# myscience/open-genie

Measured on NVIDIA H100. Metric: videotokenizer_train_step_frames_per_sec, higher is better.
Workload: dtype bf16

## Files before the change

open_genie_b200/csrc/conv3d_wgrad.cu:

```cuda
#include "og_host.cuh"
#include "og_ptx.cuh"

namespace og {
extern std::atomic<uint64_t> g_launches;

static constexpr int kWThreads = 384;
static constexpr int kVox = 64;
static constexpr int kPanelBytes = kVox * 128;
static constexpr int kTileM = 128;
static constexpr int kTileN = 256;
static constexpr int kWABytes = 2 * kPanelBytes;
static constexpr int kWBBytes = 4 * kPanelBytes;
static constexpr int kWStages = 4;
static constexpr int kSlotFloats = kTileM * kTileN;

struct WgradParams {
  int kt, kh, kw, pt, ph, pw;
  int sx_t, sx_h, sx_w;
  int bw_log2, bh_log2, bt_log2, bn_log2;
  int tiles_w, tiles_h, tiles_t;
  int num_ksteps;
  int cin, cout;
  int ncols;
  int col_tiles;
  long long units;
  int ctas;
  int granule;
  int period;
  float* dw;
  long long ld_dw;
  int vec_ok;
  float* dbias;
  int n_bias;
  float* ws;
};

__host__ __device__ __forceinline__ long long share_begin(const WgradParams& p, int b) {
  return (long long)b * (p.units / p.granule) / p.ctas * p.granule;
}

template <bool kOnes>
__device__ __forceinline__ void wgrad_mma_steps(float (&acc)[128], float (&accb)[8], int nsteps, const uint8_t* smem_a,
                                                const uint8_t* smem_b, uint32_t ones_addr, uint64_t* full,
                                                uint64_t* empty, int& s, uint32_t& ph, int lane) {
  int prev = -1;
  for (int i = 0; i < nsteps; ++i) {
    mbar_wait(&full[s], ph);
    const uint32_t a_addr = smem_u32(smem_a + s * kWABytes);
    const uint32_t b_addr = smem_u32(smem_b + s * kWBBytes);
    wgmma_fence();
#pragma unroll
    for (int k = 0; k < kVox / 16; ++k)
      wgmma_ss<256, 1, 1>(acc, gmma_desc_sw128(a_addr + k * 2048, kPanelBytes, 1024),
                          gmma_desc_sw128(b_addr + k * 2048, kPanelBytes, 1024), (i | k) != 0);
    if constexpr (kOnes) {
#pragma unroll
      for (int k = 0; k < kVox / 16; ++k)
        wgmma_ss<16, 1, 1>(accb, gmma_desc_sw128(a_addr + k * 2048, kPanelBytes, 1024),
                           gmma_desc_sw128(ones_addr, kPanelBytes, 1024), (i | k) != 0);
    }
    wgmma_commit();
    wgmma_wait<1>();
    if (prev >= 0 && lane == 0) mbar_arrive(&empty[prev]);
    prev = s;
    if (++s == kWStages) {
      s = 0;
      ph ^= 1;
    }
  }
  wgmma_wait<0>();
  if (lane == 0) mbar_arrive(&empty[prev]);
}

template <bool kBias>
__global__ void __launch_bounds__(kWThreads, 1)
    og_conv_wgrad_kernel(const __grid_constant__ CUtensorMap mapDY, const __grid_constant__ CUtensorMap mapX,
                         const WgradParams p) {
  extern __shared__ uint8_t smem_raw[];
  uint8_t* smem = reinterpret_cast<uint8_t*>((reinterpret_cast<uintptr_t>(smem_raw) + 1023) & ~uintptr_t(1023));
  uint8_t* smem_a = smem;
  uint8_t* smem_b = smem + kWStages * kWABytes;
  uint8_t* smem_ones = smem_b + kWStages * kWBBytes;
  uint64_t* full = reinterpret_cast<uint64_t*>(smem_ones + 2048);
  uint64_t* empty = full + kWStages;

  const int warp = warp_idx_uniform();
  const int lane = threadIdx.x & 31;
  const long long u_begin = share_begin(p, blockIdx.x), u_end = share_begin(p, blockIdx.x + 1);

  if (warp == 0 && lane == 0) {
    tma_prefetch_desc(&mapDY);
    tma_prefetch_desc(&mapX);
    for (int s = 0; s < kWStages; ++s) {
      mbar_init(&full[s], 1);
      mbar_init(&empty[s], 8);
    }
    fence_mbar_init();
  }
  if (kBias) {
    for (int i = threadIdx.x; i < 2048 / 4; i += kWThreads) reinterpret_cast<uint32_t*>(smem_ones)[i] = 0x3F803F80u;
    fence_proxy_async_smem();
  }
  __syncthreads();

  if (warp == 0) {
    int s = 0;
    uint32_t ph = 0;
    const int per_sample = p.tiles_w * p.tiles_h * p.tiles_t;
    long long clock = 0;
    for (long long u = u_begin; u < u_end;) {
      const int tile = (int)(u / p.num_ksteps);
      const int k0 = (int)(u - (long long)tile * p.num_ksteps);
      const int k1 = (int)min((long long)p.num_ksteps, u_end - (long long)tile * p.num_ksteps);
      u += k1 - k0;
      const int co0 = (tile / p.col_tiles) * kTileM;
      const int c0 = (tile % p.col_tiles) * kTileN;
      const int npan = min(4, (p.ncols - c0) / 64);
      int pci[4], off_w[4], off_h[4], off_t[4];
#pragma unroll
      for (int j = 0; j < 4; ++j) {
        const int c = c0 + 64 * (j < npan ? j : 0);
        const int tap = c / p.cin;
        pci[j] = c - tap * p.cin;
        off_t[j] = tap / (p.kh * p.kw) - p.pt;
        off_h[j] = (tap / p.kw) % p.kh - p.ph;
        off_w[j] = tap % p.kw - p.pw;
      }
      const uint32_t tx_bytes = (uint32_t)(kWABytes + npan * kPanelBytes);
      int ks = k0 + (int)((clock - k0 % p.period + p.period) % p.period);
      if (ks >= k1) ks = k0;
      clock += k1 - k0;
      int tn, tw, th, tt;
      auto decode = [&](int k) {
        tn = k / per_sample;
        int r = k - tn * per_sample;
        tw = r % p.tiles_w;
        r /= p.tiles_w;
        th = r % p.tiles_h;
        tt = r / p.tiles_h;
      };
      decode(ks);
      for (int i = k0; i < k1; ++i) {
        const int n = tn << p.bn_log2, w0 = tw << p.bw_log2, h0 = th << p.bh_log2, t0 = tt << p.bt_log2;
        mbar_wait(&empty[s], ph ^ 1);
        if (elect_one()) {
          mbar_expect_tx(&full[s], tx_bytes);
          uint8_t* a = smem_a + s * kWABytes;
          tma_load_5d(a, &mapDY, &full[s], co0, w0, h0, t0, n);
          tma_load_5d(a + kPanelBytes, &mapDY, &full[s], co0 + 64, w0, h0, t0, n);
          uint8_t* b = smem_b + s * kWBBytes;
          for (int j = 0; j < npan; ++j)
            tma_load_5d(b + j * kPanelBytes, &mapX, &full[s], pci[j], w0 * p.sx_w + off_w[j], h0 * p.sx_h + off_h[j],
                        t0 * p.sx_t + off_t[j], n);
        }
        __syncwarp();
        if (++s == kWStages) {
          s = 0;
          ph ^= 1;
        }
        if (++ks == k1) {
          ks = k0;
          decode(ks);
        } else if (++tw == p.tiles_w) {
          tw = 0;
          if (++th == p.tiles_h) {
            th = 0;
            if (++tt == p.tiles_t) {
              tt = 0;
              ++tn;
            }
          }
        }
      }
    }
    __syncwarp();
  } else if (warp >= 4) {
    const int wg = (warp >> 2) - 1;
    const int q = warp & 3;
    const uint32_t ones_addr = smem_u32(smem_ones);
    const uint8_t* a_wg = smem_a + wg * kPanelBytes;
    float acc[128], accb[8];
    int s = 0;
    uint32_t ph = 0;
    for (long long u = u_begin; u < u_end;) {
      const bool first = u == u_begin;
      const int tile = (int)(u / p.num_ksteps);
      const int k0 = (int)(u - (long long)tile * p.num_ksteps);
      const int k1 = (int)min((long long)p.num_ksteps, u_end - (long long)tile * p.num_ksteps);
      u += k1 - k0;
      const int co0 = (tile / p.col_tiles) * kTileM;
      const int c0 = (tile % p.col_tiles) * kTileN;
      const bool bias_tile = kBias && c0 == 0;
      if (bias_tile)
        wgrad_mma_steps<true>(acc, accb, k1 - k0, a_wg, smem_b, ones_addr, full, empty, s, ph, lane);
      else
        wgrad_mma_steps<false>(acc, accb, k1 - k0, a_wg, smem_b, ones_addr, full, empty, s, ph, lane);
      reg_fence(acc);
      reg_fence(accb);
      const bool whole = k0 == 0 && k1 == p.num_ksteps;
      const int slot = 2 * blockIdx.x + (first ? 0 : 1);
      const int c_lane = 2 * (lane & 3);
#pragma unroll
      for (int rr = 0; rr < 2; ++rr) {
        const int r = wg * 64 + q * 16 + (lane >> 2) + rr * 8;
        const int co = co0 + r;
        if (whole) {
          if (co >= p.cout) continue;
          float* row = p.dw + (long long)co * p.ld_dw + c0 + c_lane;
#pragma unroll
          for (int j = 0; j < 32; ++j) {
            if (c0 + 8 * j + c_lane >= p.ncols) continue;
            const float v0 = acc[4 * j + 2 * rr], v1 = acc[4 * j + 2 * rr + 1];
            if (p.vec_ok) {
              float2* d = reinterpret_cast<float2*>(row + 8 * j);
              const float2 o = *d;
              *d = make_float2(o.x + v0, o.y + v1);
            } else {
              row[8 * j] += v0;
              row[8 * j + 1] += v1;
            }
          }
          if (bias_tile && (lane & 3) == 0 && co < p.n_bias) p.dbias[co] += accb[2 * rr];
        } else {
          float* sl = p.ws + ((long long)slot * kTileM + r) * kTileN + c_lane;
#pragma unroll
          for (int j = 0; j < 32; ++j)
            *reinterpret_cast<float2*>(sl + 8 * j) = make_float2(acc[4 * j + 2 * rr], acc[4 * j + 2 * rr + 1]);
          if (bias_tile && (lane & 3) == 0)
            p.ws[(long long)2 * p.ctas * kSlotFloats + (long long)slot * kTileM + r] = accb[2 * rr];
        }
      }
    }
  }
}

__global__ void __launch_bounds__(256) og_wgrad_fixup_kernel(const WgradParams p) {
  const int b = blockIdx.y;
  const long long ub = share_begin(p, b + 1);
  const int tile = (int)(ub / p.num_ksteps);
  const long long t0 = (long long)tile * p.num_ksteps, t1 = t0 + p.num_ksteps;
  if (ub == t0 || share_begin(p, b) > t0) return;
  const int co0 = (tile / p.col_tiles) * kTileM, c0 = (tile % p.col_tiles) * kTileN;
  const int e = (blockIdx.x * 256 + threadIdx.x) * 4;
  const int r = e / kTileN, c = e % kTileN;
  float4 sum = make_float4(0.f, 0.f, 0.f, 0.f);
  float sumb = 0.f;
  const bool bias = p.dbias && c0 == 0 && blockIdx.x == 0 && threadIdx.x < kTileM;
  for (int sh = b; sh < p.ctas; ++sh) {
    const long long sb = share_begin(p, sh);
    if (sb >= t1) break;
    const int slot = 2 * sh + (sb >= t0 ? 0 : 1);
    const float4 v = __ldcg(reinterpret_cast<const float4*>(p.ws + (long long)slot * kSlotFloats + e));
    sum.x += v.x;
    sum.y += v.y;
    sum.z += v.z;
    sum.w += v.w;
    if (bias) sumb += __ldcg(p.ws + (long long)2 * p.ctas * kSlotFloats + (long long)slot * kTileM + threadIdx.x);
  }
  if (co0 + r < p.cout && c0 + c < p.ncols) {
    float* d = p.dw + (long long)(co0 + r) * p.ld_dw + c0 + c;
    d[0] += sum.x;
    d[1] += sum.y;
    d[2] += sum.z;
    d[3] += sum.w;
  }
  if (bias && co0 + (int)threadIdx.x < p.n_bias) p.dbias[co0 + threadIdx.x] += sumb;
}

}

static int launch_wgrad(const void* dy, int cout, const void* x, int cin, float* dw, int64_t ld_dw, int kt, int kh, int kw,
                        int pt, int ph, int pw, int N, int T, int H, int W, int Ti, int Hi, int Wi, int st, int sh, int sw,
                        void* workspace, size_t workspace_bytes, og_stream_t stream, float* dbias = nullptr,
                        int n_bias = 0) {
  using namespace og;
  OG_REQUIRE(dy && x && dw, "conv3d_wgrad: null pointer");
  OG_REQUIRE(!dbias || (n_bias > 0 && n_bias <= cout), "conv3d_wgrad: n_bias=%d must be in 1..cout", n_bias);
  OG_REQUIRE(cin > 0 && cin % 64 == 0, "conv3d_wgrad: cin=%d must be a multiple of 64", cin);
  OG_REQUIRE(cout > 0 && cout % 8 == 0, "conv3d_wgrad: cout=%d must be a multiple of 8 (TMA row stride)", cout);
  OG_REQUIRE(kt >= 1 && kh >= 1 && kw >= 1 && pt >= 0 && ph >= 0 && pw >= 0 && pt < kt && ph < kh && pw < kw,
             "conv3d_wgrad: bad kernel/padding");
  OG_REQUIRE(st >= 1 && sh >= 1 && sw >= 1 && st <= 8 && sh <= 8 && sw <= 8, "conv3d_wgrad: bad stride");
  OG_REQUIRE(N > 0 && T > 0 && H > 0 && W > 0 && Ti > 0 && Hi > 0 && Wi > 0,
             "conv3d_wgrad: extents must be positive (N=%d T=%d H=%d W=%d)", N, T, H, W);
  OG_REQUIRE(ld_dw >= (int64_t)kt * kh * kw * cin, "conv3d_wgrad: ld_dw=%lld must be >= kt*kh*kw*cin = %d",
             (long long)ld_dw, kt * kh * kw * cin);
  int bw, bh, bt, bn;
  choose_voxel_box(kVox, N, T, H, W, &bw, &bh, &bt, &bn);
  OG_REQUIRE(bw * sw <= 256 && bh * sh <= 256 && bt * st <= 256, "conv3d_wgrad: strided box exceeds the TMA limit");
  WgradParams p;
  memset(&p, 0, sizeof(p));
  p.kt = kt; p.kh = kh; p.kw = kw; p.pt = pt; p.ph = ph; p.pw = pw;
  p.sx_t = st; p.sx_h = sh; p.sx_w = sw;
  p.bw_log2 = ilog2(bw); p.bh_log2 = ilog2(bh); p.bt_log2 = ilog2(bt); p.bn_log2 = ilog2(bn);
  p.tiles_w = (W + bw - 1) / bw; p.tiles_h = (H + bh - 1) / bh; p.tiles_t = (T + bt - 1) / bt;
  p.num_ksteps = ((N + bn - 1) / bn) * p.tiles_w * p.tiles_h * p.tiles_t;
  p.cin = cin; p.cout = cout; p.dw = dw; p.ld_dw = ld_dw;
  p.ncols = kt * kh * kw * cin;
  p.col_tiles = (p.ncols + kTileN - 1) / kTileN;
  const long long tiles = (long long)((cout + kTileM - 1) / kTileM) * p.col_tiles;
  p.units = tiles * p.num_ksteps;
  const int sms = num_sms();
  p.ctas = (int)std::min<long long>(sms, std::max<long long>(1, p.units / 4));
  p.granule = 1;
  const size_t slot_bytes = (size_t)(kSlotFloats + (dbias ? kTileM : 0)) * sizeof(float);
  const long long fit = workspace ? (long long)(workspace_bytes / (2 * slot_bytes)) : 0;
  if (fit < p.ctas) {
    if (fit > tiles) {
      p.ctas = (int)fit;
    } else {
      p.granule = p.num_ksteps;
      p.ctas = (int)std::min<long long>(sms, tiles);
    }
  }
  p.period = (int)std::min<long long>(p.num_ksteps, (p.units + p.ctas - 1) / p.ctas);
  p.ws = reinterpret_cast<float*>(workspace);
  p.vec_ok = (ld_dw % 2 == 0) && ((reinterpret_cast<uintptr_t>(dw) & 7) == 0);
  p.dbias = dbias;
  p.n_bias = n_bias;
  const size_t smem_bytes = (size_t)kWStages * (kWABytes + kWBBytes) + 2048  + 1024 + 512;

  CUtensorMap mapDY, mapX;
  {
    uint64_t dims[5] = {(uint64_t)cout, (uint64_t)W, (uint64_t)H, (uint64_t)T, (uint64_t)N};
    uint64_t str[4] = {(uint64_t)cout * 2, (uint64_t)W * cout * 2, (uint64_t)H * W * cout * 2,
                       (uint64_t)T * H * W * cout * 2};
    uint32_t box[5] = {64, (uint32_t)bw, (uint32_t)bh, (uint32_t)bt, (uint32_t)bn};
    int r = make_tmap_bf16(&mapDY, dy, 5, dims, str, box);
    if (r != OG_OK) return r;
  }
  {
    uint64_t dims[5] = {(uint64_t)cin, (uint64_t)Wi, (uint64_t)Hi, (uint64_t)Ti, (uint64_t)N};
    uint64_t str[4] = {(uint64_t)cin * 2, (uint64_t)Wi * cin * 2, (uint64_t)Hi * Wi * cin * 2,
                       (uint64_t)Ti * Hi * Wi * cin * 2};
    uint32_t box[5] = {64, (uint32_t)(bw * sw), (uint32_t)(bh * sh), (uint32_t)(bt * st), (uint32_t)bn};
    uint32_t es[5] = {1, (uint32_t)sw, (uint32_t)sh, (uint32_t)st, 1};
    int r = make_tmap_bf16(&mapX, x, 5, dims, str, box, es);
    if (r != OG_OK) return r;
  }
  static bool attr_set = false;
  if (!attr_set) {
    OG_CHECK_CUDA(cudaFuncSetAttribute(og_conv_wgrad_kernel<false>, cudaFuncAttributeMaxDynamicSharedMemorySize,
                                       (int)smem_bytes));
    OG_CHECK_CUDA(cudaFuncSetAttribute(og_conv_wgrad_kernel<true>, cudaFuncAttributeMaxDynamicSharedMemorySize,
                                       (int)smem_bytes));
    attr_set = true;
  }
  if (dbias)
    og_conv_wgrad_kernel<true><<<p.ctas, kWThreads, smem_bytes, (cudaStream_t)stream>>>(mapDY, mapX, p);
  else
    og_conv_wgrad_kernel<false><<<p.ctas, kWThreads, smem_bytes, (cudaStream_t)stream>>>(mapDY, mapX, p);
  OG_CHECK_CUDA(cudaGetLastError());
  g_launches.fetch_add(1);
  if (p.granule == 1 && p.ctas > 1) {
    og_wgrad_fixup_kernel<<<dim3(kSlotFloats / 1024, p.ctas - 1), 256, 0, (cudaStream_t)stream>>>(p);
    OG_CHECK_CUDA(cudaGetLastError());
    g_launches.fetch_add(1);
  }
  return OG_OK;
}

extern "C" int og_conv3d_wgrad(const void* dy, int cout, const void* x, int cin, float* dw, int64_t ld_dw, int kt,
                               int kh, int kw, int pt, int ph, int pw, int N, int T, int H, int W, void* workspace,
                               size_t workspace_bytes, og_stream_t stream) {
  return launch_wgrad(dy, cout, x, cin, dw, ld_dw, kt, kh, kw, pt, ph, pw, N, T, H, W, T, H, W, 1, 1, 1, workspace,
                      workspace_bytes, stream);
}

extern "C" int og_conv3d_wgrad_bias(const void* dy, int cout, const void* x, int cin, float* dw, int64_t ld_dw, int kt,
                                    int kh, int kw, int pt, int ph, int pw, int N, int T, int H, int W, float* dbias,
                                    int n_bias, void* workspace, size_t workspace_bytes, og_stream_t stream) {
  if (!dbias) {
    og::set_error("conv3d_wgrad_bias: dbias is NULL");
    return OG_ERR_INVALID_ARGUMENT;
  }
  return launch_wgrad(dy, cout, x, cin, dw, ld_dw, kt, kh, kw, pt, ph, pw, N, T, H, W, T, H, W, 1, 1, 1, workspace,
                      workspace_bytes, stream, dbias, n_bias);
}

extern "C" int og_conv3d_strided_wgrad(const void* dy, int cout, const void* x, int cin, float* dw, int64_t ld_dw, int kt,
                                       int kh, int kw, int st, int sh, int sw, int pt, int ph, int pw, int N, int T, int H,
                                       int W, void* workspace, size_t workspace_bytes, og_stream_t stream) {
  OG_REQUIRE(st >= 1 && sh >= 1 && sw >= 1, "conv3d_strided_wgrad: bad stride");
  OG_REQUIRE(T + pt >= kt && H + 2 * ph >= kh && W + 2 * pw >= kw,
             "conv3d_strided_wgrad: padded input (%d,%d,%d) smaller than the kernel (%d,%d,%d)", T + pt, H + 2 * ph,
             W + 2 * pw, kt, kh, kw);
  const int To = (T + pt - kt) / st + 1, Ho = (H + 2 * ph - kh) / sh + 1, Wo = (W + 2 * pw - kw) / sw + 1;
  return launch_wgrad(dy, cout, x, cin, dw, ld_dw, kt, kh, kw, pt, ph, pw, N, To, Ho, Wo, T, H, W, st, sh, sw, workspace,
                      workspace_bytes, stream);
}
```

open_genie_b200/csrc/og_ptx.cuh:

```cuda
#pragma once
#include <cuda.h>
#include <cuda_bf16.h>
#include <cuda_runtime.h>
#include <stdint.h>

namespace og {

__device__ __forceinline__ uint32_t smem_u32(const void* p) {
  return static_cast<uint32_t>(__cvta_generic_to_shared(p));
}

__device__ __forceinline__ int warp_idx_uniform() { return __shfl_sync(0xffffffffu, (int)(threadIdx.x >> 5), 0); }
__device__ __forceinline__ bool elect_one() {
  uint32_t pred;
  asm volatile(
      "{\n"
      ".reg .pred P1;\n"
      "elect.sync _|P1, 0xffffffff;\n"
      "selp.u32 %0, 1, 0, P1;\n"
      "}\n"
      : "=r"(pred));
  return pred != 0;
}

__device__ __forceinline__ void mbar_init(uint64_t* bar, uint32_t count) {
  asm volatile("mbarrier.init.shared::cta.b64 [%0], %1;" ::"r"(smem_u32(bar)), "r"(count) : "memory");
}
__device__ __forceinline__ void fence_mbar_init() {
  asm volatile("fence.mbarrier_init.release.cluster;" ::: "memory");
}
__device__ __forceinline__ void fence_proxy_async_smem() {
  asm volatile("fence.proxy.async.shared::cta;" ::: "memory");
}
__device__ __forceinline__ void mbar_expect_tx(uint64_t* bar, uint32_t bytes) {
  asm volatile("mbarrier.arrive.expect_tx.shared::cta.b64 _, [%0], %1;" ::"r"(smem_u32(bar)), "r"(bytes)
               : "memory");
}
__device__ __forceinline__ void mbar_arrive(uint64_t* bar) {
  asm volatile("mbarrier.arrive.shared::cta.b64 _, [%0];" ::"r"(smem_u32(bar)) : "memory");
}
__device__ __forceinline__ bool mbar_try_wait(uint64_t* bar, uint32_t parity) {
  uint32_t ok;
  asm volatile(
      "{\n\t.reg .pred p;\n\t"
      "mbarrier.try_wait.parity.shared::cta.b64 p, [%1], %2;\n\t"
      "selp.u32 %0, 1, 0, p;\n\t}"
      : "=r"(ok)
      : "r"(smem_u32(bar)), "r"(parity)
      : "memory");
  return ok != 0;
}
#ifndef OG_MBAR_SPIN_LIMIT
#define OG_MBAR_SPIN_LIMIT (1u << 24)
#endif
__device__ __forceinline__ void mbar_wait(uint64_t* bar, uint32_t parity) {
  uint32_t spins = 0;
  while (!mbar_try_wait(bar, parity)) {
    if (++spins > OG_MBAR_SPIN_LIMIT) {
      __trap();
    }
  }
}

__device__ __forceinline__ void tma_prefetch_desc(const CUtensorMap* map) {
  asm volatile("prefetch.tensormap [%0];" ::"l"(map) : "memory");
}
__device__ __forceinline__ void tma_load_2d(void* smem, const CUtensorMap* map, uint64_t* bar, int c0, int c1) {
  asm volatile(
      "cp.async.bulk.tensor.2d.shared::cluster.global.mbarrier::complete_tx::bytes [%0], [%1, {%3, %4}], [%2];" ::"r"(
          smem_u32(smem)),
      "l"(map), "r"(smem_u32(bar)), "r"(c0), "r"(c1)
      : "memory");
}
__device__ __forceinline__ void tma_load_3d(void* smem, const CUtensorMap* map, uint64_t* bar, int c0, int c1, int c2) {
  asm volatile(
      "cp.async.bulk.tensor.3d.shared::cluster.global.mbarrier::complete_tx::bytes [%0], [%1, {%3, %4, %5}], "
      "[%2];" ::"r"(smem_u32(smem)),
      "l"(map), "r"(smem_u32(bar)), "r"(c0), "r"(c1), "r"(c2)
      : "memory");
}
__device__ __forceinline__ void tma_load_4d(void* smem, const CUtensorMap* map, uint64_t* bar, int c0, int c1, int c2,
                                            int c3) {
  asm volatile(
      "cp.async.bulk.tensor.4d.shared::cluster.global.mbarrier::complete_tx::bytes [%0], [%1, {%3, %4, %5, %6}], "
      "[%2];" ::"r"(smem_u32(smem)),
      "l"(map), "r"(smem_u32(bar)), "r"(c0), "r"(c1), "r"(c2), "r"(c3)
      : "memory");
}
__device__ __forceinline__ void tma_load_5d(void* smem, const CUtensorMap* map, uint64_t* bar, int c0, int c1, int c2,
                                            int c3, int c4) {
  asm volatile(
      "cp.async.bulk.tensor.5d.shared::cluster.global.mbarrier::complete_tx::bytes [%0], [%1, {%3, %4, %5, %6, %7}], "
      "[%2];" ::"r"(smem_u32(smem)),
      "l"(map), "r"(smem_u32(bar)), "r"(c0), "r"(c1), "r"(c2), "r"(c3), "r"(c4)
      : "memory");
}

__device__ __forceinline__ void wgmma_fence() { asm volatile("wgmma.fence.sync.aligned;" ::: "memory"); }
__device__ __forceinline__ void wgmma_commit() { asm volatile("wgmma.commit_group.sync.aligned;" ::: "memory"); }
template <int N>
__device__ __forceinline__ void wgmma_wait() {
  asm volatile("wgmma.wait_group.sync.aligned %0;" ::"n"(N) : "memory");
}
template <int R>
__device__ __forceinline__ void reg_fence(float (&d)[R]) {
#pragma unroll
  for (int i = 0; i < R; ++i) asm volatile("" : "+f"(d[i])::"memory");
}
__device__ __forceinline__ float ex2_approx(float x) {
  float y;
  asm("ex2.approx.ftz.f32 %0, %1;" : "=f"(y) : "f"(x));
  return y;
}

__host__ __device__ __forceinline__ uint64_t gmma_desc_sw128(uint32_t smem_addr, uint32_t lbo_bytes, uint32_t sbo_bytes) {
  uint64_t d = 0;
  d |= static_cast<uint64_t>((smem_addr >> 4) & 0x3FFF);
  d |= static_cast<uint64_t>((lbo_bytes >> 4) & 0x3FFF) << 16;
  d |= static_cast<uint64_t>((sbo_bytes >> 4) & 0x3FFF) << 32;
  d |= static_cast<uint64_t>(1) << 62;
  return d;
}

__host__ __device__ __forceinline__ uint64_t gmma_desc_sw32(uint32_t smem_addr, uint32_t lbo_bytes, uint32_t sbo_bytes) {
  uint64_t d = 0;
  d |= static_cast<uint64_t>((smem_addr >> 4) & 0x3FFF);
  d |= static_cast<uint64_t>((lbo_bytes >> 4) & 0x3FFF) << 16;
  d |= static_cast<uint64_t>((sbo_bytes >> 4) & 0x3FFF) << 32;
  d |= static_cast<uint64_t>(3) << 62;
  return d;
}

template <int TA, int TB>
__device__ __forceinline__ void wgmma_ss_n16(float (&d)[8], uint64_t adesc, uint64_t bdesc, int scale_d) {
  asm volatile(
      "{\n.reg .pred p;\nsetp.ne.b32 p, %10, 0;\n"
      "wgmma.mma_async.sync.aligned.m64n16k16.f32.bf16.bf16 {%0, %1, %2, %3, %4, %5, %6, %7}, %8, %9, p, 1, 1, %11, %12;\n}\n"
      : "+f"(d[0]), "+f"(d[1]), "+f"(d[2]), "+f"(d[3]), "+f"(d[4]), "+f"(d[5]), "+f"(d[6]), "+f"(d[7])
      : "l"(adesc), "l"(bdesc), "r"(scale_d), "n"(TA), "n"(TB));
}

template <int TA, int TB>
__device__ __forceinline__ void wgmma_ss_n32(float (&d)[16], uint64_t adesc, uint64_t bdesc, int scale_d) {
  asm volatile(
      "{\n.reg .pred p;\nsetp.ne.b32 p, %18, 0;\n"
      "wgmma.mma_async.sync.aligned.m64n32k16.f32.bf16.bf16 {%0, %1, %2, %3, %4, %5, %6, %7, %8, %9, %10, %11, %12, %13, %14, %15}, %16, %17, p, 1, 1, %19, %20;\n}\n"
      : "+f"(d[0]), "+f"(d[1]), "+f"(d[2]), "+f"(d[3]), "+f"(d[4]), "+f"(d[5]), "+f"(d[6]), "+f"(d[7]), "+f"(d[8]), "+f"(d[9]), "+f"(d[10]), "+f"(d[11]), "+f"(d[12]), "+f"(d[13]), "+f"(d[14]), "+f"(d[15])
      : "l"(adesc), "l"(bdesc), "r"(scale_d), "n"(TA), "n"(TB));
}

template <int TA, int TB>
__device__ __forceinline__ void wgmma_ss_n64(float (&d)[32], uint64_t adesc, uint64_t bdesc, int scale_d) {
  asm volatile(
      "{\n.reg .pred p;\nsetp.ne.b32 p, %34, 0;\n"
      "wgmma.mma_async.sync.aligned.m64n64k16.f32.bf16.bf16 {%0, %1, %2, %3, %4, %5, %6, %7, %8, %9, %10, %11, %12, %13, %14, %15, %16, %17, %18, %19, %20, %21, %22, %23, %24, %25, %26, %27, %28, %29, %30, %31}, %32, %33, p, 1, 1, %35, %36;\n}\n"
      : "+f"(d[0]), "+f"(d[1]), "+f"(d[2]), "+f"(d[3]), "+f"(d[4]), "+f"(d[5]), "+f"(d[6]), "+f"(d[7]), "+f"(d[8]), "+f"(d[9]), "+f"(d[10]), "+f"(d[11]), "+f"(d[12]), "+f"(d[13]), "+f"(d[14]), "+f"(d[15]), "+f"(d[16]), "+f"(d[17]), "+f"(d[18]), "+f"(d[19]), "+f"(d[20]), "+f"(d[21]), "+f"(d[22]), "+f"(d[23]), "+f"(d[24]), "+f"(d[25]), "+f"(d[26]), "+f"(d[27]), "+f"(d[28]), "+f"(d[29]), "+f"(d[30]), "+f"(d[31])
      : "l"(adesc), "l"(bdesc), "r"(scale_d), "n"(TA), "n"(TB));
}

template <int TB>
__device__ __forceinline__ void wgmma_rs_n16(float (&d)[8], const uint32_t (&a)[4], uint64_t bdesc, int scale_d) {
  asm volatile(
      "{\n.reg .pred p;\nsetp.ne.b32 p, %13, 0;\n"
      "wgmma.mma_async.sync.aligned.m64n16k16.f32.bf16.bf16 {%0, %1, %2, %3, %4, %5, %6, %7}, {%8, %9, %10, %11}, %12, p, 1, 1, %14;\n}\n"
      : "+f"(d[0]), "+f"(d[1]), "+f"(d[2]), "+f"(d[3]), "+f"(d[4]), "+f"(d[5]), "+f"(d[6]), "+f"(d[7])
      : "r"(a[0]), "r"(a[1]), "r"(a[2]), "r"(a[3]), "l"(bdesc), "r"(scale_d), "n"(TB));
}

template <int TB>
__device__ __forceinline__ void wgmma_rs_n64(float (&d)[32], const uint32_t (&a)[4], uint64_t bdesc, int scale_d) {
  asm volatile(
      "{\n.reg .pred p;\nsetp.ne.b32 p, %37, 0;\n"
      "wgmma.mma_async.sync.aligned.m64n64k16.f32.bf16.bf16 {%0, %1, %2, %3, %4, %5, %6, %7, %8, %9, %10, %11, %12, %13, %14, %15, %16, %17, %18, %19, %20, %21, %22, %23, %24, %25, %26, %27, %28, %29, %30, %31}, {%32, %33, %34, %35}, %36, p, 1, 1, %38;\n}\n"
      : "+f"(d[0]), "+f"(d[1]), "+f"(d[2]), "+f"(d[3]), "+f"(d[4]), "+f"(d[5]), "+f"(d[6]), "+f"(d[7]), "+f"(d[8]), "+f"(d[9]), "+f"(d[10]), "+f"(d[11]), "+f"(d[12]), "+f"(d[13]), "+f"(d[14]), "+f"(d[15]), "+f"(d[16]), "+f"(d[17]), "+f"(d[18]), "+f"(d[19]), "+f"(d[20]), "+f"(d[21]), "+f"(d[22]), "+f"(d[23]), "+f"(d[24]), "+f"(d[25]), "+f"(d[26]), "+f"(d[27]), "+f"(d[28]), "+f"(d[29]), "+f"(d[30]), "+f"(d[31])
      : "r"(a[0]), "r"(a[1]), "r"(a[2]), "r"(a[3]), "l"(bdesc), "r"(scale_d), "n"(TB));
}

template <int TA, int TB>
__device__ __forceinline__ void wgmma_ss_n128(float (&d)[64], uint64_t adesc, uint64_t bdesc, int scale_d) {
  asm volatile(
      "{\n.reg .pred p;\nsetp.ne.b32 p, %66, 0;\n"
      "wgmma.mma_async.sync.aligned.m64n128k16.f32.bf16.bf16 {%0, %1, %2, %3, %4, %5, %6, %7, %8, %9, %10, %11, %12, %13, %14, %15, %16, %17, %18, %19, %20, %21, %22, %23, %24, %25, %26, %27, %28, %29, %30, %31, %32, %33, %34, %35, %36, %37, %38, %39, %40, %41, %42, %43, %44, %45, %46, %47, %48, %49, %50, %51, %52, %53, %54, %55, %56, %57, %58, %59, %60, %61, %62, %63}, %64, %65, p, 1, 1, %67, %68;\n}\n"
      : "+f"(d[0]), "+f"(d[1]), "+f"(d[2]), "+f"(d[3]), "+f"(d[4]), "+f"(d[5]), "+f"(d[6]), "+f"(d[7]), "+f"(d[8]), "+f"(d[9]), "+f"(d[10]), "+f"(d[11]), "+f"(d[12]), "+f"(d[13]), "+f"(d[14]), "+f"(d[15]), "+f"(d[16]), "+f"(d[17]), "+f"(d[18]), "+f"(d[19]), "+f"(d[20]), "+f"(d[21]), "+f"(d[22]), "+f"(d[23]), "+f"(d[24]), "+f"(d[25]), "+f"(d[26]), "+f"(d[27]), "+f"(d[28]), "+f"(d[29]), "+f"(d[30]), "+f"(d[31]), "+f"(d[32]), "+f"(d[33]), "+f"(d[34]), "+f"(d[35]), "+f"(d[36]), "+f"(d[37]), "+f"(d[38]), "+f"(d[39]), "+f"(d[40]), "+f"(d[41]), "+f"(d[42]), "+f"(d[43]), "+f"(d[44]), "+f"(d[45]), "+f"(d[46]), "+f"(d[47]), "+f"(d[48]), "+f"(d[49]), "+f"(d[50]), "+f"(d[51]), "+f"(d[52]), "+f"(d[53]), "+f"(d[54]), "+f"(d[55]), "+f"(d[56]), "+f"(d[57]), "+f"(d[58]), "+f"(d[59]), "+f"(d[60]), "+f"(d[61]), "+f"(d[62]), "+f"(d[63])
      : "l"(adesc), "l"(bdesc), "r"(scale_d), "n"(TA), "n"(TB));
}

template <int TA, int TB>
__device__ __forceinline__ void wgmma_ss_n256(float (&d)[128], uint64_t adesc, uint64_t bdesc, int scale_d) {
  asm volatile(
      "{\n.reg .pred p;\nsetp.ne.b32 p, %130, 0;\n"
      "wgmma.mma_async.sync.aligned.m64n256k16.f32.bf16.bf16 {%0, %1, %2, %3, %4, %5, %6, %7, %8, %9, %10, %11, %12, %13, %14, %15, %16, %17, %18, %19, %20, %21, %22, %23, %24, %25, %26, %27, %28, %29, %30, %31, %32, %33, %34, %35, %36, %37, %38, %39, %40, %41, %42, %43, %44, %45, %46, %47, %48, %49, %50, %51, %52, %53, %54, %55, %56, %57, %58, %59, %60, %61, %62, %63, %64, %65, %66, %67, %68, %69, %70, %71, %72, %73, %74, %75, %76, %77, %78, %79, %80, %81, %82, %83, %84, %85, %86, %87, %88, %89, %90, %91, %92, %93, %94, %95, %96, %97, %98, %99, %100, %101, %102, %103, %104, %105, %106, %107, %108, %109, %110, %111, %112, %113, %114, %115, %116, %117, %118, %119, %120, %121, %122, %123, %124, %125, %126, %127}, %128, %129, p, 1, 1, %131, %132;\n}\n"
      : "+f"(d[0]), "+f"(d[1]), "+f"(d[2]), "+f"(d[3]), "+f"(d[4]), "+f"(d[5]), "+f"(d[6]), "+f"(d[7]), "+f"(d[8]), "+f"(d[9]), "+f"(d[10]), "+f"(d[11]), "+f"(d[12]), "+f"(d[13]), "+f"(d[14]), "+f"(d[15]), "+f"(d[16]), "+f"(d[17]), "+f"(d[18]), "+f"(d[19]), "+f"(d[20]), "+f"(d[21]), "+f"(d[22]), "+f"(d[23]), "+f"(d[24]), "+f"(d[25]), "+f"(d[26]), "+f"(d[27]), "+f"(d[28]), "+f"(d[29]), "+f"(d[30]), "+f"(d[31]), "+f"(d[32]), "+f"(d[33]), "+f"(d[34]), "+f"(d[35]), "+f"(d[36]), "+f"(d[37]), "+f"(d[38]), "+f"(d[39]), "+f"(d[40]), "+f"(d[41]), "+f"(d[42]), "+f"(d[43]), "+f"(d[44]), "+f"(d[45]), "+f"(d[46]), "+f"(d[47]), "+f"(d[48]), "+f"(d[49]), "+f"(d[50]), "+f"(d[51]), "+f"(d[52]), "+f"(d[53]), "+f"(d[54]), "+f"(d[55]), "+f"(d[56]), "+f"(d[57]), "+f"(d[58]), "+f"(d[59]), "+f"(d[60]), "+f"(d[61]), "+f"(d[62]), "+f"(d[63]), "+f"(d[64]), "+f"(d[65]), "+f"(d[66]), "+f"(d[67]), "+f"(d[68]), "+f"(d[69]), "+f"(d[70]), "+f"(d[71]), "+f"(d[72]), "+f"(d[73]), "+f"(d[74]), "+f"(d[75]), "+f"(d[76]), "+f"(d[77]), "+f"(d[78]), "+f"(d[79]), "+f"(d[80]), "+f"(d[81]), "+f"(d[82]), "+f"(d[83]), "+f"(d[84]), "+f"(d[85]), "+f"(d[86]), "+f"(d[87]), "+f"(d[88]), "+f"(d[89]), "+f"(d[90]), "+f"(d[91]), "+f"(d[92]), "+f"(d[93]), "+f"(d[94]), "+f"(d[95]), "+f"(d[96]), "+f"(d[97]), "+f"(d[98]), "+f"(d[99]), "+f"(d[100]), "+f"(d[101]), "+f"(d[102]), "+f"(d[103]), "+f"(d[104]), "+f"(d[105]), "+f"(d[106]), "+f"(d[107]), "+f"(d[108]), "+f"(d[109]), "+f"(d[110]), "+f"(d[111]), "+f"(d[112]), "+f"(d[113]), "+f"(d[114]), "+f"(d[115]), "+f"(d[116]), "+f"(d[117]), "+f"(d[118]), "+f"(d[119]), "+f"(d[120]), "+f"(d[121]), "+f"(d[122]), "+f"(d[123]), "+f"(d[124]), "+f"(d[125]), "+f"(d[126]), "+f"(d[127])
      : "l"(adesc), "l"(bdesc), "r"(scale_d), "n"(TA), "n"(TB));
}

template <int N, int TA, int TB>
__device__ __forceinline__ void wgmma_ss(float (&d)[N / 2], uint64_t adesc, uint64_t bdesc, int scale_d) {
  if constexpr (N == 16) wgmma_ss_n16<TA, TB>(d, adesc, bdesc, scale_d);
  else if constexpr (N == 32) wgmma_ss_n32<TA, TB>(d, adesc, bdesc, scale_d);
  else if constexpr (N == 64) wgmma_ss_n64<TA, TB>(d, adesc, bdesc, scale_d);
  else if constexpr (N == 128) wgmma_ss_n128<TA, TB>(d, adesc, bdesc, scale_d);
  else wgmma_ss_n256<TA, TB>(d, adesc, bdesc, scale_d);
}

__device__ __forceinline__ uint32_t pack_bf16x2(float lo, float hi) {
  __nv_bfloat162 v = __floats2bfloat162_rn(lo, hi);
  return *reinterpret_cast<uint32_t*>(&v);
}

__device__ __forceinline__ void stmatrix_x4_trans(uint32_t addr, uint32_t r0, uint32_t r1, uint32_t r2, uint32_t r3) {
  asm volatile("stmatrix.sync.aligned.m8n8.x4.trans.shared.b16 [%0], {%1, %2, %3, %4};" ::"r"(addr), "r"(r0), "r"(r1),
               "r"(r2), "r"(r3)
               : "memory");
}

}
```

Before: 1033.

## Trim wgrad MMA width to live panels, skip idle warpgroup, precompute fixup segments

```diff
diff --git a/open_genie_b200/csrc/conv3d_wgrad.cu b/open_genie_b200/csrc/conv3d_wgrad.cu
--- a/open_genie_b200/csrc/conv3d_wgrad.cu
+++ b/open_genie_b200/csrc/conv3d_wgrad.cu
@@ -39,10 +39,11 @@
   return (long long)b * (p.units / p.granule) / p.ctas * p.granule;
 }
 
-template <bool kOnes>
+template <bool kOnes, int kN>
 __device__ __forceinline__ void wgrad_mma_steps(float (&acc)[128], float (&accb)[8], int nsteps, const uint8_t* smem_a,
                                                 const uint8_t* smem_b, uint32_t ones_addr, uint64_t* full,
                                                 uint64_t* empty, int& s, uint32_t& ph, int lane) {
+  float(&accn)[kN / 2] = *reinterpret_cast<float(*)[kN / 2]>(&acc[0]);
   int prev = -1;
   for (int i = 0; i < nsteps; ++i) {
     mbar_wait(&full[s], ph);
@@ -51,8 +52,8 @@
     wgmma_fence();
 #pragma unroll
     for (int k = 0; k < kVox / 16; ++k)
-      wgmma_ss<256, 1, 1>(acc, gmma_desc_sw128(a_addr + k * 2048, kPanelBytes, 1024),
-                          gmma_desc_sw128(b_addr + k * 2048, kPanelBytes, 1024), (i | k) != 0);
+      wgmma_ss<kN, 1, 1>(accn, gmma_desc_sw128(a_addr + k * 2048, kPanelBytes, 1024),
+                         gmma_desc_sw128(b_addr + k * 2048, kPanelBytes, 1024), (i | k) != 0);
     if constexpr (kOnes) {
 #pragma unroll
       for (int k = 0; k < kVox / 16; ++k)
@@ -70,6 +71,96 @@
   }
   wgmma_wait<0>();
   if (lane == 0) mbar_arrive(&empty[prev]);
+}
+
+__device__ __forceinline__ void wgrad_idle_steps(int nsteps, uint64_t* full, uint64_t* empty, int& s, uint32_t& ph,
+                                                 int lane) {
+  for (int i = 0; i < nsteps; ++i) {
+    mbar_wait(&full[s], ph);
+    if (lane == 0) mbar_arrive(&empty[s]);
+    if (++s == kWStages) {
+      s = 0;
+      ph ^= 1;
+    }
+  }
+}
+
+template <bool kOnes, int kN>
+__device__ __forceinline__ void wgrad_segment(const WgradParams& p, float (&acc)[128], int k0, int k1, int co0, int c0,
+                                              int slot, int wg, int q, const uint8_t* a_wg, const uint8_t* smem_b,
+                                              uint32_t ones_addr, uint64_t* full, uint64_t* empty, int& s,
+                                              uint32_t& ph, int lane) {
+  constexpr int kJ = kN / 8;
+  constexpr int kBatch = 8;
+  float accb[8];
+  wgrad_mma_steps<kOnes, kN>(acc, accb, k1 - k0, a_wg, smem_b, ones_addr, full, empty, s, ph, lane);
+  reg_fence(acc);
+  reg_fence(accb);
+  const bool whole = k0 == 0 && k1 == p.num_ksteps;
+  const int c_lane = 2 * (lane & 3);
+  const int jn = kN < 256 ? kJ : min(kJ, (p.ncols - c0) / 8);
+#pragma unroll
+  for (int rr = 0; rr < 2; ++rr) {
+    const int r = wg * 64 + q * 16 + (lane >> 2) + rr * 8;
+    const int co = co0 + r;
+    if (co >= p.cout) continue;
+    if (whole) {
+      float* row = p.dw + (long long)co * p.ld_dw + c0 + c_lane;
+#pragma unroll
+      for (int j0 = 0; j0 < kJ; j0 += kBatch) {
+        if (j0 >= jn) break;
+        if (p.vec_ok) {
+          float2 o[kBatch];
+#pragma unroll
+          for (int j = 0; j < kBatch; ++j) o[j] = *reinterpret_cast<const float2*>(row + 8 * (j0 + j));
+#pragma unroll
+          for (int j = 0; j < kBatch; ++j)
+            *reinterpret_cast<float2*>(row + 8 * (j0 + j)) =
+                make_float2(o[j].x + acc[4 * (j0 + j) + 2 * rr], o[j].y + acc[4 * (j0 + j) + 2 * rr + 1]);
+        } else {
+          float o[2 * kBatch];
+#pragma unroll
+          for (int j = 0; j < kBatch; ++j) {
+            o[2 * j] = row[8 * (j0 + j)];
+            o[2 * j + 1] = row[8 * (j0 + j) + 1];
+          }
+#pragma unroll
+          for (int j = 0; j < kBatch; ++j) {
+            row[8 * (j0 + j)] = o[2 * j] + acc[4 * (j0 + j) + 2 * rr];
+            row[8 * (j0 + j) + 1] = o[2 * j + 1] + acc[4 * (j0 + j) + 2 * rr + 1];
+          }
+        }
+      }
+      if (kOnes && (lane & 3) == 0 && co < p.n_bias) p.dbias[co] += accb[2 * rr];
+    } else {
+      float* sl = p.ws + ((long long)slot * kTileM + r) * kTileN + c_lane;
+#pragma unroll
+      for (int j = 0; j < kJ; ++j)
+        if (j < jn)
+          *reinterpret_cast<float2*>(sl + 8 * j) = make_float2(acc[4 * j + 2 * rr], acc[4 * j + 2 * rr + 1]);
+      if (kOnes && (lane & 3) == 0)
+        p.ws[(long long)2 * p.ctas * kSlotFloats + (long long)slot * kTileM + r] = accb[2 * rr];
+    }
+  }
+}
+
+__device__ __forceinline__ void wgrad_segment_plain(const WgradParams& p, float (&acc)[128], int npan, int k0, int k1,
+                                                    int co0, int c0, int slot, int wg, int q, const uint8_t* a_wg,
+                                                    const uint8_t* smem_b, uint64_t* full, uint64_t* empty, int& s,
+                                                    uint32_t& ph, int lane) {
+  switch (npan) {
+    case 1:
+      wgrad_segment<false, 64>(p, acc, k0, k1, co0, c0, slot, wg, q, a_wg, smem_b, 0, full, empty, s, ph, lane);
+      break;
+    case 2:
+      wgrad_segment<false, 128>(p, acc, k0, k1, co0, c0, slot, wg, q, a_wg, smem_b, 0, full, empty, s, ph, lane);
+      break;
+    case 3:
+      wgrad_segment<false, 192>(p, acc, k0, k1, co0, c0, slot, wg, q, a_wg, smem_b, 0, full, empty, s, ph, lane);
+      break;
+    default:
+      wgrad_segment<false, 256>(p, acc, k0, k1, co0, c0, slot, wg, q, a_wg, smem_b, 0, full, empty, s, ph, lane);
+  }
 }
 
 template <bool kBias>
@@ -103,7 +194,9 @@
   }
   __syncthreads();
 
-  if (warp == 0) {
+  if (warp < 4) {
+    asm volatile("setmaxnreg.dec.sync.aligned.u32 40;\n" ::: "memory");
+    if (warp != 0) return;
     int s = 0;
     uint32_t ph = 0;
     const int per_sample = p.tiles_w * p.tiles_h * p.tiles_t;
@@ -174,12 +267,13 @@
       }
     }
     __syncwarp();
-  } else if (warp >= 4) {
+  } else {
+    asm volatile("setmaxnreg.inc.sync.aligned.u32 232;\n" ::: "memory");
     const int wg = (warp >> 2) - 1;
     const int q = warp & 3;
     const uint32_t ones_addr = smem_u32(smem_ones);
     const uint8_t* a_wg = smem_a + wg * kPanelBytes;
-    float acc[128], accb[8];
+    float acc[128];
     int s = 0;
     uint32_t ph = 0;
     for (long long u = u_begin; u < u_end;) {
@@ -190,81 +284,71 @@
       u += k1 - k0;
       const int co0 = (tile / p.col_tiles) * kTileM;
       const int c0 = (tile % p.col_tiles) * kTileN;
-      const bool bias_tile = kBias && c0 == 0;
-      if (bias_tile)
-        wgrad_mma_steps<true>(acc, accb, k1 - k0, a_wg, smem_b, ones_addr, full, empty, s, ph, lane);
+      const int npan = min(4, (p.ncols - c0) / 64);
+      const int slot = 2 * blockIdx.x + (first ? 0 : 1);
+      if (wg == 1 && p.cout - co0 <= 64)
+        wgrad_idle_steps(k1 - k0, full, empty, s, ph, lane);
+      else if (kBias && c0 == 0)
+        wgrad_segment<true, 256>(p, acc, k0, k1, co0, c0, slot, wg, q, a_wg, smem_b, ones_addr, full, empty, s,
+                                 ph, lane);
       else
-        wgrad_mma_steps<false>(acc, accb, k1 - k0, a_wg, smem_b, ones_addr, full, empty, s, ph, lane);
-      reg_fence(acc);
-      reg_fence(accb);
-      const bool whole = k0 == 0 && k1 == p.num_ksteps;
-      const int slot = 2 * blockIdx.x + (first ? 0 : 1);
-      const int c_lane = 2 * (lane & 3);
-#pragma unroll
-      for (int rr = 0; rr < 2; ++rr) {
-        const int r = wg * 64 + q * 16 + (lane >> 2) + rr * 8;
-        const int co = co0 + r;
-        if (whole) {
-          if (co >= p.cout) continue;
-          float* row = p.dw + (long long)co * p.ld_dw + c0 + c_lane;
-#pragma unroll
-          for (int j = 0; j < 32; ++j) {
-            if (c0 + 8 * j + c_lane >= p.ncols) continue;
-            const float v0 = acc[4 * j + 2 * rr], v1 = acc[4 * j + 2 * rr + 1];
-            if (p.vec_ok) {
-              float2* d = reinterpret_cast<float2*>(row + 8 * j);
-              const float2 o = *d;
-              *d = make_float2(o.x + v0, o.y + v1);
-            } else {
-              row[8 * j] += v0;
-              row[8 * j + 1] += v1;
-            }
-          }
-          if (bias_tile && (lane & 3) == 0 && co < p.n_bias) p.dbias[co] += accb[2 * rr];
-        } else {
-          float* sl = p.ws + ((long long)slot * kTileM + r) * kTileN + c_lane;
-#pragma unroll
-          for (int j = 0; j < 32; ++j)
-            *reinterpret_cast<float2*>(sl + 8 * j) = make_float2(acc[4 * j + 2 * rr], acc[4 * j + 2 * rr + 1]);
-          if (bias_tile && (lane & 3) == 0)
-            p.ws[(long long)2 * p.ctas * kSlotFloats + (long long)slot * kTileM + r] = accb[2 * rr];
-        }
-      }
-    }
-  }
-}
-
-__global__ void __launch_bounds__(256) og_wgrad_fixup_kernel(const WgradParams p) {
-  const int b = blockIdx.y;
-  const long long ub = share_begin(p, b + 1);
-  const int tile = (int)(ub / p.num_ksteps);
-  const long long t0 = (long long)tile * p.num_ksteps, t1 = t0 + p.num_ksteps;
-  if (ub == t0 || share_begin(p, b) > t0) return;
+        wgrad_segment_plain(p, acc, npan, k0, k1, co0, c0, slot, wg, q, a_wg, smem_b, full, empty, s, ph, lane);
+    }
+  }
+}
+
+static constexpr int kFixupMaxCtas = 256;
+struct WgradFixup {
+  int n;
+  int tile[kFixupMaxCtas];
+  short seg0[kFixupMaxCtas + 1];
+  short slot[2 * kFixupMaxCtas];
+};
+
+__global__ void __launch_bounds__(256) og_wgrad_fixup_kernel(const WgradParams p, const __grid_constant__ WgradFixup f) {
+  const int y = blockIdx.y;
+  if (y >= f.n) return;
+  const int tile = f.tile[y];
   const int co0 = (tile / p.col_tiles) * kTileM, c0 = (tile % p.col_tiles) * kTileN;
   const int e = (blockIdx.x * 256 + threadIdx.x) * 4;
   const int r = e / kTileN, c = e % kTileN;
+  const bool live = co0 + r < p.cout && c0 + c < p.ncols;
+  const bool bias = p.dbias && c0 == 0 && blockIdx.x == 0 && threadIdx.x < kTileM && co0 + (int)threadIdx.x < p.n_bias;
+  if (!live && !bias) return;
+  const float* wsb = p.ws + (long long)2 * p.ctas * kSlotFloats;
   float4 sum = make_float4(0.f, 0.f, 0.f, 0.f);
   float sumb = 0.f;
-  const bool bias = p.dbias && c0 == 0 && blockIdx.x == 0 && threadIdx.x < kTileM;
-  for (int sh = b; sh < p.ctas; ++sh) {
-    const long long sb = share_begin(p, sh);
-    if (sb >= t1) break;
-    const int slot = 2 * sh + (sb >= t0 ? 0 : 1);
-    const float4 v = __ldcg(reinterpret_cast<const float4*>(p.ws + (long long)slot * kSlotFloats + e));
-    sum.x += v.x;
-    sum.y += v.y;
-    sum.z += v.z;
-    sum.w += v.w;
-    if (bias) sumb += __ldcg(p.ws + (long long)2 * p.ctas * kSlotFloats + (long long)slot * kTileM + threadIdx.x);
-  }
-  if (co0 + r < p.cout && c0 + c < p.ncols) {
+  const int s1 = f.seg0[y + 1];
+  for (int i0 = f.seg0[y]; i0 < s1; i0 += 4) {
+    float4 v[4];
+    float vb[4];
+#pragma unroll
+    for (int i = 0; i < 4; ++i) {
+      if (i0 + i >= s1) break;
+      const int slot = f.slot[i0 + i];
+      if (live) v[i] = __ldcg(reinterpret_cast<const float4*>(p.ws + (long long)slot * kSlotFloats + e));
+      if (bias) vb[i] = __ldcg(wsb + (long long)slot * kTileM + threadIdx.x);
+    }
+#pragma unroll
+    for (int i = 0; i < 4; ++i) {
+      if (i0 + i >= s1) break;
+      if (live) {
+        sum.x += v[i].x;
+        sum.y += v[i].y;
+        sum.z += v[i].z;
+        sum.w += v[i].w;
+      }
+      if (bias) sumb += vb[i];
+    }
+  }
+  if (live) {
     float* d = p.dw + (long long)(co0 + r) * p.ld_dw + c0 + c;
     d[0] += sum.x;
     d[1] += sum.y;
     d[2] += sum.z;
     d[3] += sum.w;
   }
-  if (bias && co0 + (int)threadIdx.x < p.n_bias) p.dbias[co0 + threadIdx.x] += sumb;
+  if (bias) p.dbias[co0 + threadIdx.x] += sumb;
 }
 
 }
@@ -314,6 +398,8 @@
     }
   }
   p.period = (int)std::min<long long>(p.num_ksteps, (p.units + p.ctas - 1) / p.ctas);
+  OG_REQUIRE(p.ctas <= kFixupMaxCtas, "conv3d_wgrad: %d shares exceed the fixup's tile list (%d)", p.ctas,
+             kFixupMaxCtas);
   p.ws = reinterpret_cast<float*>(workspace);
   p.vec_ok = (ld_dw % 2 == 0) && ((reinterpret_cast<uintptr_t>(dw) & 7) == 0);
   p.dbias = dbias;
@@ -353,7 +439,24 @@
   OG_CHECK_CUDA(cudaGetLastError());
   g_launches.fetch_add(1);
   if (p.granule == 1 && p.ctas > 1) {
-    og_wgrad_fixup_kernel<<<dim3(kSlotFloats / 1024, p.ctas - 1), 256, 0, (cudaStream_t)stream>>>(p);
+    WgradFixup f;
+    f.n = 0;
+    int ns = 0;
+    for (int b = 0; b + 1 < p.ctas; ++b) {
+      const long long ub = share_begin(p, b + 1);
+      const int tile = (int)(ub / p.num_ksteps);
+      const long long t0 = (long long)tile * p.num_ksteps, t1 = t0 + p.num_ksteps;
+      if (ub == t0 || share_begin(p, b) > t0) continue;
+      f.tile[f.n] = tile;
+      f.seg0[f.n++] = (short)ns;
+      for (int sh = b; sh < p.ctas; ++sh) {
+        const long long sb = share_begin(p, sh);
+        if (sb >= t1) break;
+        f.slot[ns++] = (short)(2 * sh + (sb >= t0 ? 0 : 1));
+      }
+    }
+    f.seg0[f.n] = (short)ns;
+    og_wgrad_fixup_kernel<<<dim3(kSlotFloats / 1024, std::max(f.n, 1)), 256, 0, (cudaStream_t)stream>>>(p, f);
     OG_CHECK_CUDA(cudaGetLastError());
     g_launches.fetch_add(1);
   }
diff --git a/open_genie_b200/csrc/og_ptx.cuh b/open_genie_b200/csrc/og_ptx.cuh
--- a/open_genie_b200/csrc/og_ptx.cuh
+++ b/open_genie_b200/csrc/og_ptx.cuh
@@ -186,6 +186,15 @@
 }
 
 template <int TA, int TB>
+__device__ __forceinline__ void wgmma_ss_n192(float (&d)[96], uint64_t adesc, uint64_t bdesc, int scale_d) {
+  asm volatile(
+      "{\n.reg .pred p;\nsetp.ne.b32 p, %98, 0;\n"
+      "wgmma.mma_async.sync.aligned.m64n192k16.f32.bf16.bf16 {%0, %1, %2, %3, %4, %5, %6, %7, %8, %9, %10, %11, %12, %13, %14, %15, %16, %17, %18, %19, %20, %21, %22, %23, %24, %25, %26, %27, %28, %29, %30, %31, %32, %33, %34, %35, %36, %37, %38, %39, %40, %41, %42, %43, %44, %45, %46, %47, %48, %49, %50, %51, %52, %53, %54, %55, %56, %57, %58, %59, %60, %61, %62, %63, %64, %65, %66, %67, %68, %69, %70, %71, %72, %73, %74, %75, %76, %77, %78, %79, %80, %81, %82, %83, %84, %85, %86, %87, %88, %89, %90, %91, %92, %93, %94, %95}, %96, %97, p, 1, 1, %99, %100;\n}\n"
+      : "+f"(d[0]), "+f"(d[1]), "+f"(d[2]), "+f"(d[3]), "+f"(d[4]), "+f"(d[5]), "+f"(d[6]), "+f"(d[7]), "+f"(d[8]), "+f"(d[9]), "+f"(d[10]), "+f"(d[11]), "+f"(d[12]), "+f"(d[13]), "+f"(d[14]), "+f"(d[15]), "+f"(d[16]), "+f"(d[17]), "+f"(d[18]), "+f"(d[19]), "+f"(d[20]), "+f"(d[21]), "+f"(d[22]), "+f"(d[23]), "+f"(d[24]), "+f"(d[25]), "+f"(d[26]), "+f"(d[27]), "+f"(d[28]), "+f"(d[29]), "+f"(d[30]), "+f"(d[31]), "+f"(d[32]), "+f"(d[33]), "+f"(d[34]), "+f"(d[35]), "+f"(d[36]), "+f"(d[37]), "+f"(d[38]), "+f"(d[39]), "+f"(d[40]), "+f"(d[41]), "+f"(d[42]), "+f"(d[43]), "+f"(d[44]), "+f"(d[45]), "+f"(d[46]), "+f"(d[47]), "+f"(d[48]), "+f"(d[49]), "+f"(d[50]), "+f"(d[51]), "+f"(d[52]), "+f"(d[53]), "+f"(d[54]), "+f"(d[55]), "+f"(d[56]), "+f"(d[57]), "+f"(d[58]), "+f"(d[59]), "+f"(d[60]), "+f"(d[61]), "+f"(d[62]), "+f"(d[63]), "+f"(d[64]), "+f"(d[65]), "+f"(d[66]), "+f"(d[67]), "+f"(d[68]), "+f"(d[69]), "+f"(d[70]), "+f"(d[71]), "+f"(d[72]), "+f"(d[73]), "+f"(d[74]), "+f"(d[75]), "+f"(d[76]), "+f"(d[77]), "+f"(d[78]), "+f"(d[79]), "+f"(d[80]), "+f"(d[81]), "+f"(d[82]), "+f"(d[83]), "+f"(d[84]), "+f"(d[85]), "+f"(d[86]), "+f"(d[87]), "+f"(d[88]), "+f"(d[89]), "+f"(d[90]), "+f"(d[91]), "+f"(d[92]), "+f"(d[93]), "+f"(d[94]), "+f"(d[95])
+      : "l"(adesc), "l"(bdesc), "r"(scale_d), "n"(TA), "n"(TB));
+}
+
+template <int TA, int TB>
 __device__ __forceinline__ void wgmma_ss_n256(float (&d)[128], uint64_t adesc, uint64_t bdesc, int scale_d) {
   asm volatile(
       "{\n.reg .pred p;\nsetp.ne.b32 p, %130, 0;\n"
@@ -200,6 +209,7 @@
   else if constexpr (N == 32) wgmma_ss_n32<TA, TB>(d, adesc, bdesc, scale_d);
   else if constexpr (N == 64) wgmma_ss_n64<TA, TB>(d, adesc, bdesc, scale_d);
   else if constexpr (N == 128) wgmma_ss_n128<TA, TB>(d, adesc, bdesc, scale_d);
+  else if constexpr (N == 192) wgmma_ss_n192<TA, TB>(d, adesc, bdesc, scale_d);
   else wgmma_ss_n256<TA, TB>(d, adesc, bdesc, scale_d);
 }
 
```

After: 1052, median of 6. +1.9%, better.
